# little-little-point-cloud-group/buildingSegment

Measured on AMD Instinct MI355X. Metric: Mpoints/s segmented (kNN+normal+label), higher is better.
Workload: dtype int32 coordinates / f64 normals; 1 GPU; urban_50m; points_per_gpu=50000000, k=16, max_nn=50, rg_mode=0, largest_plane=135921, seed_attempts=6951, fallback_queries=0, rg_rounds=25, validation_rejects=1, tie_rows=971975, parallelism=1 GPU, whole path

## Files before the change

buildingsegment_amd/csrc/bs_grid.hip:

```cpp
#include <hipcub/hipcub.hpp>

#include <algorithm>
#include <climits>
#include <cmath>
#include <cstdio>
#include <cstdlib>

#include "bs_common.h"

namespace bs {

namespace {

__global__ void bbox_kernel(const int32_t* __restrict__ xyz, int64_t n, int32_t* __restrict__ mnmx)
{
  int mn[3] = {INT_MAX, INT_MAX, INT_MAX}, mx[3] = {INT_MIN, INT_MIN, INT_MIN};
  for (int64_t i = blockIdx.x * (int64_t)blockDim.x + threadIdx.x; i < n;
       i += (int64_t)gridDim.x * blockDim.x) {
#pragma unroll
    for (int a = 0; a < 3; a++) {
      int v = xyz[3 * i + a];
      mn[a] = min(mn[a], v);
      mx[a] = max(mx[a], v);
    }
// ... 81 lines not shown
    t[i].end = 0;
  }
}

__global__ void table_insert_kernel(const uint64_t* __restrict__ ukeys, const int32_t* __restrict__ ucnt,
                                    const int32_t* __restrict__ ustart, int32_t ncell, int morton,
                                    CellEntry* table, uint32_t hmask)
{
  int32_t c = blockIdx.x * blockDim.x + threadIdx.x;
  if (c >= ncell)
    return;
  uint64_t k = ukeys[c];
  if (morton)
    k = pack_cell(compact21(k), compact21(k >> 1), compact21(k >> 2));
  uint32_t h = hash_cell(k) & hmask;
  for (;;) {
    unsigned long long prev =
        atomicCAS((unsigned long long*)&table[h].key, ~0ull, (unsigned long long)k);
    if (prev == ~0ull)
      break;
    h = (h + 1) & hmask;
  }
  table[h].start = ustart[c];
  table[h].end = ustart[c] + ucnt[c];
}

__global__ void gather_sorted_kernel(const int32_t* __restrict__ xyz, const int32_t* __restrict__ gidx,
                                     const int32_t* __restrict__ order, int64_t n, int4* __restrict__ spts)
{
  int64_t s = blockIdx.x * (int64_t)blockDim.x + threadIdx.x;
  if (s >= n)
    return;
  int32_t i = order[s];
  int4 v;
  v.x = xyz[3 * (int64_t)i];
  v.y = xyz[3 * (int64_t)i + 1];
  v.z = xyz[3 * (int64_t)i + 2];
  v.w = gidx ? gidx[i] : i;
  spts[s] = v;
}

inline int grid_blocks(int64_t n, int bs) { return (int)((n + bs - 1) / bs); }

}

static int morton_key_bits(int64_t ext, int cell)
{
  int bits = 1;
  while (((int64_t)1 << bits) < ext / cell + 1)
    bits++;
  return std::min(63, 3 * bits);
}

static int sort_count_keys(bs_ctx* ctx, int64_t n, int end_bit, int64_t* ncell)
{
  hipStream_t st = ctx->stream;
  uint64_t* kin = ctx->keys_in.as<uint64_t>();
  uint64_t* kout = ctx->keys_out.as<uint64_t>();
  size_t tb = 0;
  BS_HIP(ctx, hipcub::DeviceRadixSort::SortKeys(nullptr, tb, kin, kout, (int)n, 0, end_bit, st));
  BS_HIP(ctx, ctx->cub_tmp.reserve(tb));
  BS_HIP(ctx, hipcub::DeviceRadixSort::SortKeys(ctx->cub_tmp.p, tb, kin, kout, (int)n, 0, end_bit, st));
  unsigned long long* cnt = ctx->misc.as<unsigned long long>() + 8;
  BS_HIP(ctx, hipMemsetAsync(cnt, 0, sizeof(unsigned long long), st));
  count_heads_kernel<<<std::min(grid_blocks(n, 256), 1024), 256, 0, st>>>(kout, n, cnt);
  unsigned long long h = 0;
  BS_HIP(ctx, hipMemcpyAsync(&h, cnt, sizeof h, hipMemcpyDeviceToHost, st));
  BS_HIP(ctx, hipStreamSynchronize(st));
  *ncell = (int64_t)h;
  return BS_OK;
}

static int count_cells(bs_ctx* ctx, const int32_t* d_xyz, int64_t n, const int mn[3], int cell, int64_t ext,
                       int64_t* ncell)
{
  cellkey_kernel<<<grid_blocks(n, 256), 256, 0, ctx->stream>>>(d_xyz, n, mn[0], mn[1], mn[2], cell, 1,
                                                               ctx->keys_in.as<uint64_t>(), nullptr);
  return sort_count_keys(ctx, n, morton_key_bits(ext, cell), ncell);
}

int build_grid(bs_ctx* ctx, const int32_t* d_xyz, const int32_t* d_gidx, int64_t n, double radius,
               int k, int cell_hint, GridDev* out)
{
  hipStream_t st = ctx->stream;
  if (n <= 0 || n >= (int64_t)INT_MAX - 64)
    return fail(ctx, BS_ERR_INVALID, "point count out of range");
  BS_HIP(ctx, ctx->misc.reserve(256));
  BS_HIP(ctx, ctx->keys_in.reserve(sizeof(uint64_t) * n));
  BS_HIP(ctx, ctx->keys_out.reserve(sizeof(uint64_t) * n));
  BS_HIP(ctx, ctx->vals_in.reserve(sizeof(int32_t) * n));
  BS_HIP(ctx, ctx->vals_out.reserve(sizeof(int32_t) * n));

  int32_t init[6] = {INT_MAX, INT_MAX, INT_MAX, INT_MIN, INT_MIN, INT_MIN};
  int32_t* d_mnmx = ctx->misc.as<int32_t>();
  BS_HIP(ctx, hipMemcpyAsync(d_mnmx, init, sizeof init, hipMemcpyHostToDevice, st));
  bbox_kernel<<<std::min(grid_blocks(n, 256), 512), 256, 0, st>>>(d_xyz, n, d_mnmx);
  int32_t bb[6];
  BS_HIP(ctx, hipMemcpyAsync(bb, d_mnmx, sizeof bb, hipMemcpyDeviceToHost, st));
  BS_HIP(ctx, hipStreamSynchronize(st));
  const int32_t LIM = 1 << 23;
  for (int a = 0; a < 3; a++)
    if (bb[a] <= -LIM || bb[3 + a] >= LIM)
      return fail(ctx, BS_ERR_RANGE, "coordinates must satisfy |c| < 2^23 mm (8.4 km): shift the cloud to its bounding-box origin first "
                                     "(bs_shift_to_origin_dev, or the buildingSeg constructor as TMC3.cpp:210 does)");

  int64_t ext = 1;
  for (int a = 0; a < 3; a++)
    ext = std::max<int64_t>(ext, (int64_t)bb[3 + a] - bb[a] + 1);
  int cell = cell_hint > 0 ? cell_hint : (int)std::max(1.0, std::ceil(radius));
  if (cell_hint <= 0) {
    const double target = std::max(4.0, 0.5 * k);
    const int cmin = cell;
    for (int it = 0; it < 4; it++) {
      int64_t nc = 0;
      int rc = count_cells(ctx, d_xyz, n, bb, cell, ext, &nc);
      if (rc != BS_OK)
        return rc;
      double occ = (double)n / (double)std::max<int64_t>(nc, 1);
      if (occ >= 0.7 * target && occ <= 1.6 * target)
        break;
      double f = std::sqrt(target / occ);
      f = std::min(4.0, std::max(0.25, f));
      int ncell = (int)std::floor(cell * f + 0.5);
      ncell = std::max(ncell, cmin);
      if (ncell == cell || (int64_t)ncell > ext)
        break;
      cell = ncell;
    }
  }
  while (ext / cell + 1 >= (1 << 21))
    cell *= 2;

  uint64_t* kin = ctx->keys_in.as<uint64_t>();
  uint64_t* kout = ctx->keys_out.as<uint64_t>();
  int32_t* vin = ctx->vals_in.as<int32_t>();
  int32_t* vout = ctx->vals_out.as<int32_t>();
  static const int morton = []() {
    const char* e = getenv("BS_GRID_ORDER");
    return (e && e[0] == 'r') ? 0 : 1;
  }();
  cellkey_kernel<<<grid_blocks(n, 256), 256, 0, st>>>(d_xyz, n, bb[0], bb[1], bb[2], cell, morton, kin, vin);
  size_t tb = 0;
  const int end_bit = morton ? morton_key_bits(ext, cell) : 63;
  BS_HIP(ctx, hipcub::DeviceRadixSort::SortPairs(nullptr, tb, kin, kout, vin, vout, (int)n, 0, end_bit, st));
  BS_HIP(ctx, ctx->cub_tmp.reserve(tb));
  BS_HIP(ctx, hipcub::DeviceRadixSort::SortPairs(ctx->cub_tmp.p, tb, kin, kout, vin, vout, (int)n, 0, end_bit, st));

  BS_HIP(ctx, ctx->uniq_keys.reserve(sizeof(uint64_t) * n));
  BS_HIP(ctx, ctx->uniq_cnt.reserve(sizeof(int32_t) * 2 * n));
  uint64_t* ukeys = ctx->uniq_keys.as<uint64_t>();
  int32_t* ucnt = ctx->uniq_cnt.as<int32_t>();
  int32_t* ustart = ucnt + n;
  int32_t* d_nruns = ctx->misc.as<int32_t>() + 32;
  tb = 0;
  BS_HIP(ctx, hipcub::DeviceRunLengthEncode::Encode(nullptr, tb, kout, ukeys, ucnt, d_nruns, (int)n, st));
  BS_HIP(ctx, ctx->cub_tmp.reserve(tb));
  BS_HIP(ctx, hipcub::DeviceRunLengthEncode::Encode(ctx->cub_tmp.p, tb, kout, ukeys, ucnt, d_nruns, (int)n, st));
  int32_t nruns = 0;
  BS_HIP(ctx, hipMemcpyAsync(&nruns, d_nruns, sizeof nruns, hipMemcpyDeviceToHost, st));
  BS_HIP(ctx, hipStreamSynchronize(st));
  if (nruns <= 0)
    return fail(ctx, BS_ERR_INTERNAL, "grid: no occupied cells");
  tb = 0;
  BS_HIP(ctx, hipcub::DeviceScan::ExclusiveSum(nullptr, tb, ucnt, ustart, nruns, st));
  BS_HIP(ctx, ctx->cub_tmp.reserve(tb));
  BS_HIP(ctx, hipcub::DeviceScan::ExclusiveSum(ctx->cub_tmp.p, tb, ucnt, ustart, nruns, st));

  uint32_t hs = 64;
  while (hs < (uint32_t)nruns * 2u)
    hs <<= 1;
  BS_HIP(ctx, ctx->table.reserve(sizeof(CellEntry) * (size_t)hs));
  CellEntry* table = ctx->table.as<CellEntry>();
  table_clear_kernel<<<(hs + 255) / 256, 256, 0, st>>>(table, hs);
  table_insert_kernel<<<(nruns + 255) / 256, 256, 0, st>>>(ukeys, ucnt, ustart, nruns, morton, table, hs - 1);

  BS_HIP(ctx, ctx->spts.reserve(sizeof(int4) * n));
  gather_sorted_kernel<<<grid_blocks(n, 256), 256, 0, st>>>(d_xyz, d_gidx, vout, n, ctx->spts.as<int4>());
  BS_HIP(ctx, hipGetLastError());

  out->mn[0] = bb[0];
  out->mn[1] = bb[1];
  out->mn[2] = bb[2];
  for (int a = 0; a < 3; a++)
    out->dim[a] = (int32_t)(((int64_t)bb[3 + a] - bb[a]) / cell + 1);
  out->cell = cell;
  out->hmask = hs - 1;
  out->table = table;
  out->spts = ctx->spts.as<int4>();
  out->slocal = vout;
  out->n = n;
  ctx->order_n = n;
  ctx->order_xyz = d_xyz;
  return BS_OK;
}

int bbox_dev(bs_ctx* ctx, const int32_t* d_xyz, int64_t n, int32_t bb[6])
{
  hipStream_t st = ctx->stream;
  BS_HIP(ctx, ctx->misc.reserve(256));
// ... 162 lines not shown
                       const int32_t* d_mnmx)
{
  tile_shift_kernel<<<grid_blocks(n, 256), 256, 0, ctx->stream>>>(d_xyz, n, d_off, n_tiles, d_mnmx);
}

int build_grid_tiled(bs_ctx* ctx, const int32_t* d_xyz, const int32_t* d_off, const std::vector<int64_t>& off,
                     double radius, int k, int cell_hint, TiledGridDev* out)
{
  hipStream_t st = ctx->stream;
  const int32_t nt = (int32_t)off.size() - 1;
  const int64_t n = off[nt];
  if (nt < 1 || n <= 0 || n >= (int64_t)INT_MAX - 64)
    return fail(ctx, BS_ERR_INVALID, "point count out of range");
  BS_HIP(ctx, ctx->misc.reserve(256));
  BS_HIP(ctx, ctx->keys_in.reserve(sizeof(uint64_t) * n));
  BS_HIP(ctx, ctx->keys_out.reserve(sizeof(uint64_t) * n));
  BS_HIP(ctx, ctx->vals_in.reserve(sizeof(int32_t) * n));
  BS_HIP(ctx, ctx->vals_out.reserve(sizeof(int32_t) * n));
  BS_HIP(ctx, ctx->bt[BT_MNMX].reserve(sizeof(int32_t) * 6 * nt));
  BS_HIP(ctx, ctx->bt[BT_DESC].reserve(sizeof(TileDesc) * nt));

  std::vector<int32_t> bb;
  int rc = tile_bbox_dev(ctx, d_xyz, d_off, off, ctx->bt[BT_MNMX].as<int32_t>(), bb);
  if (rc != BS_OK)
    return rc;
  const int32_t LIM = 1 << 23;
  int64_t ext = 1;
  for (int32_t t = 0; t < nt; t++)
    for (int a = 0; a < 3; a++) {
      if (bb[6 * t + a] <= -LIM || bb[6 * t + 3 + a] >= LIM) {
        char msg[256];
        snprintf(msg, sizeof msg, "tile %d: coordinates must satisfy |c| < 2^23 mm (8.4 km): shift every tile to its "
                                  "bounding-box origin first (bs_shift_tiles_to_origin_dev)", t);
        return fail(ctx, BS_ERR_RANGE, msg);
      }
      ext = std::max<int64_t>(ext, (int64_t)bb[6 * t + 3 + a] - bb[6 * t + a] + 1);
    }
  int tbits = 0;
  while (((int64_t)1 << tbits) < nt)
    tbits++;
  auto fits = [&](int64_t c) { return ext / c + 1 < (1 << 21) && tbits + morton_key_bits(ext, (int)c) <= 63; };
  std::vector<TileDesc> desc(nt);
  auto upload_desc = [&](int c) -> hipError_t {
    for (int32_t t = 0; t < nt; t++)
      for (int a = 0; a < 3; a++) {
        desc[t].mn[a] = bb[6 * t + a];
        desc[t].dim[a] = (int32_t)(((int64_t)bb[6 * t + 3 + a] - bb[6 * t + a]) / c + 1);
      }
    return hipMemcpyAsync(ctx->bt[BT_DESC].p, desc.data(), sizeof(TileDesc) * nt, hipMemcpyHostToDevice, st);
  };
  BS_HIP(ctx, upload_desc(1));
  const TileDesc* d_desc = ctx->bt[BT_DESC].as<TileDesc>();

  int cell = cell_hint > 0 ? cell_hint : (int)std::max(1.0, std::ceil(radius));
  if (cell_hint <= 0) {
    const double target = std::max(4.0, 0.5 * k);
    const int cmin = cell;
    for (int it = 0; it < 4 && fits(cell); it++) {
      const int mb = morton_key_bits(ext, cell);
      tiled_cellkey_kernel<<<grid_blocks(n, 256), 256, 0, st>>>(d_xyz, n, d_off, nt, d_desc, cell, mb,
                                                                ctx->keys_in.as<uint64_t>(), nullptr);
      int64_t nc = 0;
      rc = sort_count_keys(ctx, n, tbits + mb, &nc);
      if (rc != BS_OK)
        return rc;
      double occ = (double)n / (double)std::max<int64_t>(nc, 1);
      if (occ >= 0.7 * target && occ <= 1.6 * target)
        break;
      double f = std::sqrt(target / occ);
      f = std::min(4.0, std::max(0.25, f));
      int ncell = (int)std::floor(cell * f + 0.5);
      ncell = std::max(ncell, cmin);
      if (ncell == cell || (int64_t)ncell > ext)
        break;
      cell = ncell;
    }
  }
  while (!fits(cell))
    cell *= 2;
  const int mbits = morton_key_bits(ext, cell);
  BS_HIP(ctx, upload_desc(cell));

  uint64_t* kin = ctx->keys_in.as<uint64_t>();
  uint64_t* kout = ctx->keys_out.as<uint64_t>();
  int32_t* vin = ctx->vals_in.as<int32_t>();
  int32_t* vout = ctx->vals_out.as<int32_t>();
  tiled_cellkey_kernel<<<grid_blocks(n, 256), 256, 0, st>>>(d_xyz, n, d_off, nt, d_desc, cell, mbits, kin, vin);
  size_t tb = 0;
  const int end_bit = tbits + mbits;
  BS_HIP(ctx, hipcub::DeviceRadixSort::SortPairs(nullptr, tb, kin, kout, vin, vout, (int)n, 0, end_bit, st));
  BS_HIP(ctx, ctx->cub_tmp.reserve(tb));
  BS_HIP(ctx, hipcub::DeviceRadixSort::SortPairs(ctx->cub_tmp.p, tb, kin, kout, vin, vout, (int)n, 0, end_bit, st));

  BS_HIP(ctx, ctx->uniq_keys.reserve(sizeof(uint64_t) * n));
  BS_HIP(ctx, ctx->uniq_cnt.reserve(sizeof(int32_t) * 2 * n));
  uint64_t* ukeys = ctx->uniq_keys.as<uint64_t>();
  int32_t* ucnt = ctx->uniq_cnt.as<int32_t>();
  int32_t* ustart = ucnt + n;
  int32_t* d_nruns = ctx->misc.as<int32_t>() + 32;
  tb = 0;
  BS_HIP(ctx, hipcub::DeviceRunLengthEncode::Encode(nullptr, tb, kout, ukeys, ucnt, d_nruns, (int)n, st));
  BS_HIP(ctx, ctx->cub_tmp.reserve(tb));
  BS_HIP(ctx, hipcub::DeviceRunLengthEncode::Encode(ctx->cub_tmp.p, tb, kout, ukeys, ucnt, d_nruns, (int)n, st));
  int32_t nruns = 0;
  BS_HIP(ctx, hipMemcpyAsync(&nruns, d_nruns, sizeof nruns, hipMemcpyDeviceToHost, st));
  BS_HIP(ctx, hipStreamSynchronize(st));
  if (nruns <= 0)
    return fail(ctx, BS_ERR_INTERNAL, "grid: no occupied cells");
  tb = 0;
  BS_HIP(ctx, hipcub::DeviceScan::ExclusiveSum(nullptr, tb, ucnt, ustart, nruns, st));
  BS_HIP(ctx, ctx->cub_tmp.reserve(tb));
  BS_HIP(ctx, hipcub::DeviceScan::ExclusiveSum(ctx->cub_tmp.p, tb, ucnt, ustart, nruns, st));

  uint32_t hs = 64;
  while (hs < (uint32_t)nruns * 2u)
    hs <<= 1;
  BS_HIP(ctx, ctx->table.reserve(sizeof(CellEntry) * (size_t)hs));
  CellEntry* table = ctx->table.as<CellEntry>();
  table_clear_kernel<<<(hs + 255) / 256, 256, 0, st>>>(table, hs);
  table_insert_kernel<<<(nruns + 255) / 256, 256, 0, st>>>(ukeys, ucnt, ustart, nruns, 0, table, hs - 1);

  BS_HIP(ctx, ctx->spts.reserve(sizeof(int4) * n));
  gather_sorted_kernel<<<grid_blocks(n, 256), 256, 0, st>>>(d_xyz, nullptr, vout, n, ctx->spts.as<int4>());
  BS_HIP(ctx, hipGetLastError());

  for (int a = 0; a < 3; a++) {
    out->mn[a] = desc[0].mn[a];
    out->dim[a] = desc[0].dim[a];
  }
  out->cell = cell;
  out->hmask = hs - 1;
  out->table = table;
  out->spts = ctx->spts.as<int4>();
  out->slocal = vout;
  out->n = n;
  out->tiles = d_desc;
  out->tile_off = d_off;
  out->n_tiles = nt;
  out->mbits = mbits;
  ctx->order_n = n;
  ctx->order_xyz = d_xyz;
  return BS_OK;
}

}
// ... 1 lines not shown
```

buildingsegment_amd/csrc/bs_knn.hip:

```cpp
#include <cstdlib>
#include <type_traits>

#include "bs_common.h"
#include "bs_normal.h"

namespace bs {

namespace {

constexpr int BS_FAST_RINGS = 2;
constexpr int BS_GENERAL_RINGS = 6;

template <bool TILED>
using GridOf = std::conditional_t<TILED, TiledGridDev, GridDev>;

template <bool TILED>
__device__ inline uint64_t cell_key(uint32_t cx, uint32_t cy, uint32_t cz, uint64_t kbase)
{
  if constexpr (TILED)
    return kbase | morton_cell(cx, cy, cz);
  else
    return pack_cell(cx, cy, cz);
}

__device__ inline void tile_enter(TiledGridDev& g, int64_t s, uint64_t& kbase, int64_t& lo, int64_t& hi)
{
  const int32_t t = tile_of(g.tile_off, g.n_tiles, s);
  const TileDesc d = g.tiles[t];
#pragma unroll
  for (int a = 0; a < 3; a++) {
    g.mn[a] = d.mn[a];
    g.dim[a] = d.dim[a];
  }
  kbase = (uint64_t)t << g.mbits;
  lo = g.tile_off[t];
  hi = g.tile_off[t + 1];
}

template <bool TILED = false>
__device__ inline bool cell_lookup(const GridDev& g, uint32_t cx, uint32_t cy, uint32_t cz, int& start,
                                   int& end, uint64_t kbase = 0)
{
  const uint64_t k = cell_key<TILED>(cx, cy, cz, kbase);
  uint32_t h = hash_cell(k) & g.hmask;
  for (;;) {
    const int4 raw = *reinterpret_cast<const int4*>(&g.table[h]);
    const uint64_t ek = (uint64_t)(uint32_t)raw.x | ((uint64_t)(uint32_t)raw.y << 32);
    if (ek == k) {
      start = raw.z;
      end = raw.w;
      return true;
    }
// ... 135 lines not shown
#pragma unroll
  for (int j = 0; j < KC; j++)
    kth_final = (j == K - 1) ? best[j] : kth_final;
  if (!done || m.n > max_nn || kth_final == ~0ull) {
    const int slot = atomicAdd(fb_count, 1);
    fb_list[slot] = (int32_t)s;
    return;
  }
  int32_t* row = neigh + (int64_t)(loc - q_begin) * K;
#pragma unroll
  for (int j = 0; j < KC; j++)
    if (j < K)
      row[j] = (int32_t)(uint32_t)best[j];
  if (npos) {
    int32_t* prow = npos + s * K;
#pragma unroll
    for (int j = 0; j < KC; j++)
      if (j < K)
        prow[j] = bpos[j];
  }
  if (normals) {
    const V3 nv = normal_from_moments(m);
    double* o = normals + 3 * (int64_t)(loc - q_begin);
    o[0] = nv.x;
    o[1] = nv.y;
    o[2] = nv.z;
    if (npos) {
      double* po = pnorm_of(npos, g.n, K) + 3 * s;
      po[0] = nv.x;
      po[1] = nv.y;
      po[2] = nv.z;
    }
  }
  if (cert_r2 && (kth_final >> 32) >= cert_r2)
    atomicAdd(uncert, 1ull);
  if (tie_rows) {
    bool tie = false;
    uint64_t next = runner;
#pragma unroll
    for (int j = 0; j + 1 < KC; j++) {
      tie = tie || (j + 1 < K && (best[j] >> 32) == (best[j + 1] >> 32));
      next = (j + 1 == K) ? best[j + 1] : next;
    }
    tie = tie || (next != ~0ull && (next >> 32) == (kth_final >> 32));
    if (tie)
      atomicAdd(tie_rows, 1ull);
  }
}

#ifndef BS_KNN_CAP4
#define BS_KNN_CAP4 0
#endif
constexpr int KBUF = 8;

template <int KC, bool REL32, bool TILED = false>
__global__ __launch_bounds__(256) __attribute__((amdgpu_waves_per_eu(KC == 16 && REL32 && BS_KNN_CAP4 ? 4 : 2))) void knn_fast2_kernel(GridOf<TILED> g, int64_t q_begin, int64_t q_end, int K,
                                                       int max_nn, double r2, int32_t* __restrict__ neigh,
                                                       double* __restrict__ normals,
                                                       int32_t* __restrict__ fb_list,
                                                       int32_t* __restrict__ fb_count, uint64_t cert_r2,
                                                       unsigned long long* __restrict__ uncert,
                                                       int32_t* __restrict__ npos, unsigned long long* __restrict__ tie_rows)
{
  const int64_t s = xcd_logical_block() * (int64_t)blockDim.x + threadIdx.x;
  if (s >= g.n)
    return;
  const int32_t loc = g.slocal[s];
  if (loc < q_begin || loc >= q_end)
    return;
  uint64_t kbase = 0;
  if constexpr (TILED) {
    int64_t lo, hi;
    tile_enter(g, s, kbase, lo, hi);
  }
  uint64_t runner = ~0ull;
  const int4 P = g.spts[s];
  const int q[3] = {P.x, P.y, P.z};
  const int ci[3] = {(int)((uint32_t)(P.x - g.mn[0]) / (uint32_t)g.cell),
                     (int)((uint32_t)(P.y - g.mn[1]) / (uint32_t)g.cell),
                     (int)((uint32_t)(P.z - g.mn[2]) / (uint32_t)g.cell)};
  __shared__ uint32_t blo[KBUF][256], bhi[KBUF][256];
  __shared__ int bps[KBUF][256];
  int nbuf = 0;
  uint64_t best[KC];
  int bpos[KC];
#pragma unroll
  for (int j = 0; j < KC; j++) {
    best[j] = ~0ull;
    bpos[j] = 0;
  }
  Moments m = {};
  int rsx = 0, rsy = 0, rsz = 0, rsxx = 0, rsyy = 0, rszz = 0, rsxy = 0, rsxz = 0, rsyz = 0, rn = 0;
  bool done = false;
  auto flush = [&]() {
    uint64_t bk[KBUF];
    int bp[KBUF];
#pragma unroll
    for (int i = 0; i < KBUF; i++) {
      const bool have = i < nbuf;
      bk[i] = have ? (((uint64_t)bhi[i][threadIdx.x] << 32) | blo[i][threadIdx.x]) : ~0ull;
      bp[i] = have ? bps[i][threadIdx.x] : 0;
    }
    nbuf = 0;
#define BS_CE(ka, pa, kb, pb)            \
  do {                                   \
    const bool sw_ = (kb) < (ka);        \
    const uint64_t tk_ = (ka);           \
    const int tp_ = (pa);                \
    (ka) = sw_ ? (kb) : (ka);            \
    (pa) = sw_ ? (pb) : (pa);            \
    (kb) = sw_ ? tk_ : (kb);             \
    (pb) = sw_ ? tp_ : (pb);             \
  } while (0)
    constexpr int net[19][2] = {{0, 1}, {2, 3}, {4, 5}, {6, 7}, {0, 2}, {1, 3}, {4, 6}, {5, 7}, {1, 2}, {5, 6},
                                {0, 4}, {3, 7}, {1, 5}, {2, 6}, {1, 4}, {3, 6}, {2, 4}, {3, 5}, {3, 4}};
#pragma unroll
    for (int c = 0; c < 19; c++)
      BS_CE(bk[net[c][0]], bp[net[c][0]], bk[net[c][1]], bp[net[c][1]]);
#pragma unroll
    for (int i = 0; i < KBUF; i++)
      BS_CE(best[KC - KBUF + i], bpos[KC - KBUF + i], bk[KBUF - 1 - i], bp[KBUF - 1 - i]);
#pragma unroll
    for (int i = 0; i < KBUF; i++)
      runner = bk[i] < runner ? bk[i] : runner;
#pragma unroll
    for (int d = KC / 2; d >= 1; d >>= 1) {
#pragma unroll
      for (int i = 0; i < KC; i++)
        if ((i & d) == 0)
          BS_CE(best[i], bpos[i], best[i + d], bpos[i + d]);
    }
#undef BS_CE
  };
  for (int rho = 0; rho <= BS_FAST_RINGS && !done; rho++) {
    for (int dz = -rho; dz <= rho; dz++) {
      const int cz = ci[2] + dz;
      if (cz < 0 || cz >= g.dim[2])
        continue;
      for (int dy = -rho; dy <= rho; dy++) {
        const int cy = ci[1] + dy;
        if (cy < 0 || cy >= g.dim[1])
          continue;
        const bool face = (dz == -rho || dz == rho || dy == -rho || dy == rho);
        const int step = face ? 1 : (rho > 0 ? 2 * rho : 1);
        for (int dx0 = -rho; dx0 <= rho; dx0 += 3 * step) {
          int4 raw[3];
          uint64_t ck[3];
          uint32_t hh[3];
          bool want[3];
#pragma unroll
          for (int u = 0; u < 3; u++) {
            const int dx = dx0 + u * step;
            const int cx = ci[0] + dx;
            want[u] = dx <= rho && cx >= 0 && cx < g.dim[0];
            ck[u] = cell_key<TILED>((uint32_t)(want[u] ? cx : ci[0]), (uint32_t)cy, (uint32_t)cz, kbase);
            hh[u] = hash_cell(ck[u]) & g.hmask;
            raw[u] = *reinterpret_cast<const int4*>(&g.table[hh[u]]);
          }
          int cs3[3], ce3[3];
#pragma unroll
          for (int u = 0; u < 3; u++) {
            cs3[u] = 0;
            ce3[u] = 0;
            if (!want[u])
              continue;
            for (;;) {
              const uint64_t ek = (uint64_t)(uint32_t)raw[u].x | ((uint64_t)(uint32_t)raw[u].y << 32);
              if (ek == ck[u]) {
                cs3[u] = raw[u].z;
                ce3[u] = raw[u].w;
                break;
              }
              if (ek == ~0ull)
                break;
              hh[u] = (hh[u] + 1) & g.hmask;
              raw[u] = *reinterpret_cast<const int4*>(&g.table[hh[u]]);
            }
          }
#pragma unroll 1
          for (int u = 0; u < 3; u++) {
            const int cs = u == 0 ? cs3[0] : (u == 1 ? cs3[1] : cs3[2]);
            const int ce = u == 0 ? ce3[0] : (u == 1 ? ce3[1] : ce3[2]);
            for (int t0 = cs; t0 < ce; t0 += 4) {
              int4 cc[4];
#pragma unroll
              for (int v = 0; v < 4; v++)
                cc[v] = g.spts[t0 + v < ce ? t0 + v : ce - 1];
#pragma unroll
              for (int v = 0; v < 4; v++) {
                const int t = t0 + v;
                const int4 c = cc[v];
                const int ex = c.x - q[0], ey = c.y - q[1], ez = c.z - q[2];
                const uint32_t d2 = (uint32_t)(ex * ex) + (uint32_t)(ey * ey) + (uint32_t)(ez * ez);
                const uint64_t key = ((uint64_t)d2 << 32) | (uint32_t)c.w;
                const bool real = t < ce;
                if (real && key < best[KC - 1]) {
                  blo[nbuf][threadIdx.x] = (uint32_t)key;
                  bhi[nbuf][threadIdx.x] = d2;
                  bps[nbuf][threadIdx.x] = t;
                  nbuf++;
                } else if (real) {
                  runner = key < runner ? key : runner;
                }
                if (__ballot(nbuf == KBUF))
                  flush();
                if (real && (double)d2 < r2) {
                  if constexpr (REL32) {
                    rsx += ex;
                    rsy += ey;
                    rsz += ez;
                    rsxx += __mul24(ex, ex);
                    rsyy += __mul24(ey, ey);
                    rszz += __mul24(ez, ez);
                    rsxy += __mul24(ex, ey);
                    rsxz += __mul24(ex, ez);
                    rsyz += __mul24(ey, ez);
                    rn += 1;
                  } else {
                    moments_add(m, c.x, c.y, c.z);
                  }
                }
              }
            }
          }
        }
      }
    }
    if (__ballot(nbuf > 0))
      flush();
    uint64_t R2;
    const bool bounded = guaranteed_radius(g, q, ci, rho, R2);
    if (!bounded) {
      done = true;
    } else {
      uint64_t kth = ~0ull;
#pragma unroll
      for (int j = 0; j < KC; j++)
        kth = (j == K - 1) ? best[j] : kth;
      const bool knn_ok = kth != ~0ull && (kth >> 32) < R2;
      const bool nrm_ok = (double)R2 >= r2;
      done = knn_ok && nrm_ok;
    }
  }
  uint64_t kth_final = ~0ull;
#pragma unroll
  for (int j = 0; j < KC; j++)
    kth_final = (j == K - 1) ? best[j] : kth_final;
  if constexpr (REL32) {
    const int64_t n64 = rn, qx = q[0], qy = q[1], qz = q[2];
    m.n = rn;
    m.sx = n64 * qx + rsx;
    m.sy = n64 * qy + rsy;
    m.sz = n64 * qz + rsz;
    m.sxx = (uint64_t)(n64 * qx * qx + 2 * qx * rsx + rsxx);
    m.syy = (uint64_t)(n64 * qy * qy + 2 * qy * rsy + rsyy);
    m.szz = (uint64_t)(n64 * qz * qz + 2 * qz * rsz + rszz);
    m.sxy = n64 * qx * qy + qx * rsy + qy * rsx + rsxy;
    m.sxz = n64 * qx * qz + qx * rsz + qz * rsx + rsxz;
    m.syz = n64 * qy * qz + qy * rsz + qz * rsy + rsyz;
  }
  if (!done || m.n > max_nn || kth_final == ~0ull) {
    const int slot = atomicAdd(fb_count, 1);
    fb_list[slot] = (int32_t)s;
    return;
  }
  int32_t* row = neigh + (int64_t)(loc - q_begin) * K;
#pragma unroll
  for (int j = 0; j < KC; j++)
    if (j < K)
      row[j] = (int32_t)(uint32_t)best[j];
  if (npos) {
    int32_t* prow = npos + s * K;
#pragma unroll
    for (int j = 0; j < KC; j++)
      if (j < K)
        prow[j] = bpos[j];
  }
  if (normals) {
    const V3 nv = normal_from_moments(m);
    double* o = normals + 3 * (int64_t)(loc - q_begin);
    o[0] = nv.x;
    o[1] = nv.y;
    o[2] = nv.z;
    if (npos) {
      double* po = pnorm_of(npos, g.n, K) + 3 * s;
      po[0] = nv.x;
      po[1] = nv.y;
      po[2] = nv.z;
    }
  }
  if (cert_r2 && (kth_final >> 32) >= cert_r2)
    atomicAdd(uncert, 1ull);
  if (tie_rows) {
    bool tie = false;
    uint64_t next = runner;
#pragma unroll
// ... 321 lines not shown
        bool tie = count > K && bd2[K] == bd2[K - 1];
        for (int j = 0; j + 1 < K; j++)
          tie = tie || bd2[j] == bd2[j + 1];
        if (tie)
          atomicAdd(tie_rows, 1ull);
      }
    }
    __syncthreads();
  }
}

__global__ void mark_all_kernel(GridDev g, int64_t q_begin, int64_t q_end, int32_t* fb_list,
                                int32_t* fb_count)
{
  const int64_t s = blockIdx.x * (int64_t)blockDim.x + threadIdx.x;
  if (s >= g.n)
    return;
  const int32_t loc = g.slocal[s];
  if (loc < q_begin || loc >= q_end)
    return;
  fb_list[atomicAdd(fb_count, 1)] = (int32_t)s;
}

}

template <bool TILED>
static int launch_knn(bs_ctx* ctx, const GridOf<TILED>& g, int64_t q_begin, int64_t q_end, const bs_params& p,
                      int32_t* d_neigh, double* d_normals, double cert_radius, int64_t* n_uncertified, int32_t* d_npos)
{
  hipStream_t st = ctx->stream;
  const int64_t n = g.n;
  BS_HIP(ctx, ctx->fb_list.reserve(sizeof(int32_t) * (2 * n + 32)));
  int32_t* fb_list = ctx->fb_list.as<int32_t>() + 16;
  int32_t* fb_count = ctx->fb_list.as<int32_t>();
  int32_t* fb2_list = fb_list + n + 16;
  int32_t* fb2_count = ctx->fb_list.as<int32_t>() + 2;
  unsigned long long* uncert = (unsigned long long*)(ctx->fb_list.as<int32_t>() + 4);
  unsigned long long* tie_rows = (unsigned long long*)(ctx->fb_list.as<int32_t>() + 8);
  BS_HIP(ctx, hipMemsetAsync(ctx->fb_list.p, 0, 64, st));
  const double r2 = p.radius * p.radius;
  uint64_t cert_r2 = 0;
  if (cert_radius > 0) {
    double c2 = cert_radius * cert_radius;
    cert_r2 = c2 >= 1.8e19 ? ~0ull : (uint64_t)std::ceil(c2);
    if (cert_r2 == 0)
      cert_r2 = 1;
  }
  const int blocks = (int)((n + 255) / 256);
  const int xblocks = xcd_grid(blocks);
  const bool fast_ok = (int64_t)g.cell * (2 * BS_FAST_RINGS + 1) <= 37500;
  if (fast_ok) {
    const bool buffered = getenv("BS_KNN_BUFFERED") ? atoi(getenv("BS_KNN_BUFFERED")) != 0 : true;
    const bool rel32 = r2 <= 32761.0 && !getenv("BS_KNN_MOMENTS64");
    if (buffered && p.k <= 16 && rel32)
      knn_fast2_kernel<16, true, TILED><<<xblocks, 256, 0, st>>>(g, q_begin, q_end, p.k, p.max_nn, r2, d_neigh, d_normals,
                                                         fb_list, fb_count, cert_r2, uncert, d_npos, tie_rows);
    else if (buffered && p.k <= 16)
      knn_fast2_kernel<16, false, TILED><<<xblocks, 256, 0, st>>>(g, q_begin, q_end, p.k, p.max_nn, r2, d_neigh, d_normals,
                                                          fb_list, fb_count, cert_r2, uncert, d_npos, tie_rows);
    else if (buffered && rel32)
      knn_fast2_kernel<32, true, TILED><<<xblocks, 256, 0, st>>>(g, q_begin, q_end, p.k, p.max_nn, r2, d_neigh, d_normals,
                                                         fb_list, fb_count, cert_r2, uncert, d_npos, tie_rows);
    else if (buffered)
      knn_fast2_kernel<32, false, TILED><<<xblocks, 256, 0, st>>>(g, q_begin, q_end, p.k, p.max_nn, r2, d_neigh, d_normals,
                                                          fb_list, fb_count, cert_r2, uncert, d_npos, tie_rows);
    else if (p.k <= 16)
      knn_fast_kernel<16, TILED><<<xblocks, 256, 0, st>>>(g, q_begin, q_end, p.k, p.max_nn, r2, d_neigh, d_normals,
                                                  fb_list, fb_count, cert_r2, uncert, d_npos, tie_rows);
    else
      knn_fast_kernel<32, TILED><<<xblocks, 256, 0, st>>>(g, q_begin, q_end, p.k, p.max_nn, r2, d_neigh, d_normals,
                                                  fb_list, fb_count, cert_r2, uncert, d_npos, tie_rows);
  } else {
    mark_all_kernel<<<blocks, 256, 0, st>>>(g, q_begin, q_end, fb_list, fb_count);
  }
  if (getenv("BS_KNN_GENERAL_THREAD")) {
    knn_general_kernel<TILED><<<1024, 64, 0, st>>>(g, q_begin, p.k, p.max_nn, r2, d_neigh, d_normals, fb_list, fb_count, cert_r2,
                                            uncert, d_npos, tie_rows);
  } else {
    knn_general_wave_kernel<TILED><<<8192, 64, 0, st>>>(g, q_begin, p.k, p.max_nn, r2, d_neigh, d_normals, fb_list, fb_count, cert_r2,
                                                 uncert, d_npos, tie_rows, fb2_list, fb2_count);
    knn_general_kernel<TILED><<<1024, 64, 0, st>>>(g, q_begin, p.k, p.max_nn, r2, d_neigh, d_normals, fb2_list, fb2_count, cert_r2,
                                            uncert, d_npos, tie_rows);
  }
  BS_HIP(ctx, hipGetLastError());
  int32_t hb[4];
  BS_HIP(ctx, hipMemcpyAsync(hb, ctx->fb_list.p, sizeof hb, hipMemcpyDeviceToHost, st));
  unsigned long long hu = 0, ht = 0;
  BS_HIP(ctx, hipMemcpyAsync(&hu, uncert, sizeof hu, hipMemcpyDeviceToHost, st));
  BS_HIP(ctx, hipMemcpyAsync(&ht, tie_rows, sizeof ht, hipMemcpyDeviceToHost, st));
  BS_HIP(ctx, hipStreamSynchronize(st));
  ctx->tm.n_fallback_queries = hb[0];
  ctx->tm.tie_rows = (int64_t)ht;
  if (n_uncertified)
    *n_uncertified = (int64_t)hu;
  return BS_OK;
}

int launch_knn_normals(bs_ctx* ctx, const GridDev& g, int64_t q_begin, int64_t q_end, const bs_params& p,
                       int32_t* d_neigh, double* d_normals, double cert_radius, int64_t* n_uncertified, int32_t* d_npos)
{
  return launch_knn<false>(ctx, g, q_begin, q_end, p, d_neigh, d_normals, cert_radius, n_uncertified, d_npos);
}

int launch_knn_normals_tiled(bs_ctx* ctx, const TiledGridDev& g, const bs_params& p, int32_t* d_neigh,
                             double* d_normals, int32_t* d_npos)
{
  return launch_knn<true>(ctx, g, 0, g.n, p, d_neigh, d_normals, 0.0, nullptr, d_npos);
}

}
```

Before: 199.2 Mpoints/s.

## Stream ring-1 kNN cells as one candidate queue and reuse grid-sizing sort

In the buffered kNN kernel, the ring-1 neighborhood is processed per z-slab. All 9 hash lookups are issued up front, the non-empty cell ranges are stored in shared memory, and their candidates are consumed as one continuous stream of 4-wide batches that cross cell boundaries. This is meant to cut the wave divergence and idle lanes caused by short per-cell loops, at the cost of extra shared memory and a changed occupancy hint (waves_per_eu 3). Separately, grid building now sorts key/value pairs from the second cell-size probe onward, so if the last probe's cell size is the final one, the final cellkey and radix sort are skipped. The in-radius test also switches from a double comparison to a precomputed integer threshold.

```diff
diff --git a/buildingsegment_amd/csrc/bs_grid.hip b/buildingsegment_amd/csrc/bs_grid.hip
--- a/buildingsegment_amd/csrc/bs_grid.hip
+++ b/buildingsegment_amd/csrc/bs_grid.hip
@@ -157,15 +157,23 @@
   return std::min(63, 3 * bits);
 }
 
-static int sort_count_keys(bs_ctx* ctx, int64_t n, int end_bit, int64_t* ncell)
+static int sort_count_keys(bs_ctx* ctx, int64_t n, int end_bit, int64_t* ncell, bool pairs)
 {
   hipStream_t st = ctx->stream;
   uint64_t* kin = ctx->keys_in.as<uint64_t>();
   uint64_t* kout = ctx->keys_out.as<uint64_t>();
+  int32_t* vin = ctx->vals_in.as<int32_t>();
+  int32_t* vout = ctx->vals_out.as<int32_t>();
   size_t tb = 0;
-  BS_HIP(ctx, hipcub::DeviceRadixSort::SortKeys(nullptr, tb, kin, kout, (int)n, 0, end_bit, st));
-  BS_HIP(ctx, ctx->cub_tmp.reserve(tb));
-  BS_HIP(ctx, hipcub::DeviceRadixSort::SortKeys(ctx->cub_tmp.p, tb, kin, kout, (int)n, 0, end_bit, st));
+  if (pairs) {
+    BS_HIP(ctx, hipcub::DeviceRadixSort::SortPairs(nullptr, tb, kin, kout, vin, vout, (int)n, 0, end_bit, st));
+    BS_HIP(ctx, ctx->cub_tmp.reserve(tb));
+    BS_HIP(ctx, hipcub::DeviceRadixSort::SortPairs(ctx->cub_tmp.p, tb, kin, kout, vin, vout, (int)n, 0, end_bit, st));
+  } else {
+    BS_HIP(ctx, hipcub::DeviceRadixSort::SortKeys(nullptr, tb, kin, kout, (int)n, 0, end_bit, st));
+    BS_HIP(ctx, ctx->cub_tmp.reserve(tb));
+    BS_HIP(ctx, hipcub::DeviceRadixSort::SortKeys(ctx->cub_tmp.p, tb, kin, kout, (int)n, 0, end_bit, st));
+  }
   unsigned long long* cnt = ctx->misc.as<unsigned long long>() + 8;
   BS_HIP(ctx, hipMemsetAsync(cnt, 0, sizeof(unsigned long long), st));
   count_heads_kernel<<<std::min(grid_blocks(n, 256), 1024), 256, 0, st>>>(kout, n, cnt);
@@ -177,11 +185,18 @@
 }
 
 static int count_cells(bs_ctx* ctx, const int32_t* d_xyz, int64_t n, const int mn[3], int cell, int64_t ext,
-                       int64_t* ncell)
+                       int64_t* ncell, bool pairs)
 {
   cellkey_kernel<<<grid_blocks(n, 256), 256, 0, ctx->stream>>>(d_xyz, n, mn[0], mn[1], mn[2], cell, 1,
-                                                               ctx->keys_in.as<uint64_t>(), nullptr);
-  return sort_count_keys(ctx, n, morton_key_bits(ext, cell), ncell);
+                                                               ctx->keys_in.as<uint64_t>(),
+                                                               pairs ? ctx->vals_in.as<int32_t>() : nullptr);
+  return sort_count_keys(ctx, n, morton_key_bits(ext, cell), ncell, pairs);
+}
+
+static bool grid_reuse_on()
+{
+  const char* e = getenv("BS_GRID_REUSE");
+  return !e || atoi(e) != 0;
 }
 
 int build_grid(bs_ctx* ctx, const int32_t* d_xyz, const int32_t* d_gidx, int64_t n, double radius,
@@ -212,15 +227,23 @@
   int64_t ext = 1;
   for (int a = 0; a < 3; a++)
     ext = std::max<int64_t>(ext, (int64_t)bb[3 + a] - bb[a] + 1);
+  static const int morton = []() {
+    const char* e = getenv("BS_GRID_ORDER");
+    return (e && e[0] == 'r') ? 0 : 1;
+  }();
+  const bool reuse = morton && grid_reuse_on();
+  int sorted_cell = 0;
   int cell = cell_hint > 0 ? cell_hint : (int)std::max(1.0, std::ceil(radius));
   if (cell_hint <= 0) {
     const double target = std::max(4.0, 0.5 * k);
     const int cmin = cell;
     for (int it = 0; it < 4; it++) {
       int64_t nc = 0;
-      int rc = count_cells(ctx, d_xyz, n, bb, cell, ext, &nc);
+      const bool pairs = reuse && it >= 1;
+      int rc = count_cells(ctx, d_xyz, n, bb, cell, ext, &nc, pairs);
       if (rc != BS_OK)
         return rc;
+      sorted_cell = pairs ? cell : 0;
       double occ = (double)n / (double)std::max<int64_t>(nc, 1);
       if (occ >= 0.7 * target && occ <= 1.6 * target)
         break;
@@ -240,16 +263,14 @@
   uint64_t* kout = ctx->keys_out.as<uint64_t>();
   int32_t* vin = ctx->vals_in.as<int32_t>();
   int32_t* vout = ctx->vals_out.as<int32_t>();
-  static const int morton = []() {
-    const char* e = getenv("BS_GRID_ORDER");
-    return (e && e[0] == 'r') ? 0 : 1;
-  }();
-  cellkey_kernel<<<grid_blocks(n, 256), 256, 0, st>>>(d_xyz, n, bb[0], bb[1], bb[2], cell, morton, kin, vin);
   size_t tb = 0;
-  const int end_bit = morton ? morton_key_bits(ext, cell) : 63;
-  BS_HIP(ctx, hipcub::DeviceRadixSort::SortPairs(nullptr, tb, kin, kout, vin, vout, (int)n, 0, end_bit, st));
-  BS_HIP(ctx, ctx->cub_tmp.reserve(tb));
-  BS_HIP(ctx, hipcub::DeviceRadixSort::SortPairs(ctx->cub_tmp.p, tb, kin, kout, vin, vout, (int)n, 0, end_bit, st));
+  if (sorted_cell != cell) {
+    cellkey_kernel<<<grid_blocks(n, 256), 256, 0, st>>>(d_xyz, n, bb[0], bb[1], bb[2], cell, morton, kin, vin);
+    const int end_bit = morton ? morton_key_bits(ext, cell) : 63;
+    BS_HIP(ctx, hipcub::DeviceRadixSort::SortPairs(nullptr, tb, kin, kout, vin, vout, (int)n, 0, end_bit, st));
+    BS_HIP(ctx, ctx->cub_tmp.reserve(tb));
+    BS_HIP(ctx, hipcub::DeviceRadixSort::SortPairs(ctx->cub_tmp.p, tb, kin, kout, vin, vout, (int)n, 0, end_bit, st));
+  }
 
   BS_HIP(ctx, ctx->uniq_keys.reserve(sizeof(uint64_t) * n));
   BS_HIP(ctx, ctx->uniq_cnt.reserve(sizeof(int32_t) * 2 * n));
@@ -518,18 +539,23 @@
   BS_HIP(ctx, upload_desc(1));
   const TileDesc* d_desc = ctx->bt[BT_DESC].as<TileDesc>();
 
+  const bool reuse = grid_reuse_on();
+  int sorted_cell = 0;
   int cell = cell_hint > 0 ? cell_hint : (int)std::max(1.0, std::ceil(radius));
   if (cell_hint <= 0) {
     const double target = std::max(4.0, 0.5 * k);
     const int cmin = cell;
     for (int it = 0; it < 4 && fits(cell); it++) {
       const int mb = morton_key_bits(ext, cell);
+      const bool pairs = reuse && it >= 1;
       tiled_cellkey_kernel<<<grid_blocks(n, 256), 256, 0, st>>>(d_xyz, n, d_off, nt, d_desc, cell, mb,
-                                                                ctx->keys_in.as<uint64_t>(), nullptr);
+                                                                ctx->keys_in.as<uint64_t>(),
+                                                                pairs ? ctx->vals_in.as<int32_t>() : nullptr);
       int64_t nc = 0;
-      rc = sort_count_keys(ctx, n, tbits + mb, &nc);
+      rc = sort_count_keys(ctx, n, tbits + mb, &nc, pairs);
       if (rc != BS_OK)
         return rc;
+      sorted_cell = pairs ? cell : 0;
       double occ = (double)n / (double)std::max<int64_t>(nc, 1);
       if (occ >= 0.7 * target && occ <= 1.6 * target)
         break;
@@ -551,12 +577,14 @@
   uint64_t* kout = ctx->keys_out.as<uint64_t>();
   int32_t* vin = ctx->vals_in.as<int32_t>();
   int32_t* vout = ctx->vals_out.as<int32_t>();
-  tiled_cellkey_kernel<<<grid_blocks(n, 256), 256, 0, st>>>(d_xyz, n, d_off, nt, d_desc, cell, mbits, kin, vin);
   size_t tb = 0;
-  const int end_bit = tbits + mbits;
-  BS_HIP(ctx, hipcub::DeviceRadixSort::SortPairs(nullptr, tb, kin, kout, vin, vout, (int)n, 0, end_bit, st));
-  BS_HIP(ctx, ctx->cub_tmp.reserve(tb));
-  BS_HIP(ctx, hipcub::DeviceRadixSort::SortPairs(ctx->cub_tmp.p, tb, kin, kout, vin, vout, (int)n, 0, end_bit, st));
+  if (sorted_cell != cell) {
+    tiled_cellkey_kernel<<<grid_blocks(n, 256), 256, 0, st>>>(d_xyz, n, d_off, nt, d_desc, cell, mbits, kin, vin);
+    const int end_bit = tbits + mbits;
+    BS_HIP(ctx, hipcub::DeviceRadixSort::SortPairs(nullptr, tb, kin, kout, vin, vout, (int)n, 0, end_bit, st));
+    BS_HIP(ctx, ctx->cub_tmp.reserve(tb));
+    BS_HIP(ctx, hipcub::DeviceRadixSort::SortPairs(ctx->cub_tmp.p, tb, kin, kout, vin, vout, (int)n, 0, end_bit, st));
+  }
 
   BS_HIP(ctx, ctx->uniq_keys.reserve(sizeof(uint64_t) * n));
   BS_HIP(ctx, ctx->uniq_cnt.reserve(sizeof(int32_t) * 2 * n));
diff --git a/buildingsegment_amd/csrc/bs_knn.hip b/buildingsegment_amd/csrc/bs_knn.hip
--- a/buildingsegment_amd/csrc/bs_knn.hip
+++ b/buildingsegment_amd/csrc/bs_knn.hip
@@ -1,3 +1,6 @@
+#include <algorithm>
+#include <cmath>
+#include <cstdio>
 #include <cstdlib>
 #include <type_traits>
 
@@ -239,10 +242,16 @@
 #define BS_KNN_CAP4 0
 #endif
 constexpr int KBUF = 8;
-
-template <int KC, bool REL32, bool TILED = false>
-__global__ __launch_bounds__(256) __attribute__((amdgpu_waves_per_eu(KC == 16 && REL32 && BS_KNN_CAP4 ? 4 : 2))) void knn_fast2_kernel(GridOf<TILED> g, int64_t q_begin, int64_t q_end, int K,
-                                                       int max_nn, double r2, int32_t* __restrict__ neigh,
+#ifndef BS_KNN_PROBE_GROUP
+#define BS_KNN_PROBE_GROUP 3
+#endif
+#ifdef BS_PROBE
+__device__ unsigned long long g_knn_probe[8];
+#endif
+
+template <int KC, bool REL32, bool TILED = false, bool STREAM = false>
+__global__ __launch_bounds__(256) __attribute__((amdgpu_waves_per_eu(KC == 16 && REL32 && BS_KNN_CAP4 ? 4 : (KC == 16 && REL32 && STREAM ? 3 : 2)))) void knn_fast2_kernel(GridOf<TILED> g, int64_t q_begin, int64_t q_end, int K,
+                                                       int max_nn, double r2, uint32_t r2le, int32_t* __restrict__ neigh,
                                                        double* __restrict__ normals,
                                                        int32_t* __restrict__ fb_list,
                                                        int32_t* __restrict__ fb_count, uint64_t cert_r2,
@@ -268,6 +277,7 @@
                      (int)((uint32_t)(P.z - g.mn[2]) / (uint32_t)g.cell)};
   __shared__ uint32_t blo[KBUF][256], bhi[KBUF][256];
   __shared__ int bps[KBUF][256];
+  __shared__ int srs[STREAM ? 9 : 1][STREAM ? 256 : 1], sre[STREAM ? 9 : 1][STREAM ? 256 : 1];
   int nbuf = 0;
   uint64_t best[KC];
   int bpos[KC];
@@ -279,7 +289,7 @@
   Moments m = {};
   int rsx = 0, rsy = 0, rsz = 0, rsxx = 0, rsyy = 0, rszz = 0, rsxy = 0, rsxz = 0, rsyz = 0, rn = 0;
   bool done = false;
-  auto flush = [&]() {
+  auto flush = [&]() __attribute__((always_inline)) {
     uint64_t bk[KBUF];
     int bp[KBUF];
 #pragma unroll
@@ -319,8 +329,154 @@
     }
 #undef BS_CE
   };
+  auto cand_slot = [&](const int4 c, const int t, const bool real) __attribute__((always_inline)) {
+    const int ex = c.x - q[0], ey = c.y - q[1], ez = c.z - q[2];
+    const uint32_t d2 = (uint32_t)(ex * ex) + (uint32_t)(ey * ey) + (uint32_t)(ez * ez);
+    const uint64_t key = ((uint64_t)d2 << 32) | (uint32_t)c.w;
+    if (real && key < best[KC - 1]) {
+      blo[nbuf][threadIdx.x] = (uint32_t)key;
+      bhi[nbuf][threadIdx.x] = d2;
+      bps[nbuf][threadIdx.x] = t;
+      nbuf++;
+    } else if (real) {
+      runner = key < runner ? key : runner;
+    }
+    if (__ballot(nbuf == KBUF))
+      flush();
+    if (real && d2 <= r2le) {
+      if constexpr (REL32) {
+        rsx += ex;
+        rsy += ey;
+        rsz += ez;
+        rsxx += __mul24(ex, ex);
+        rsyy += __mul24(ey, ey);
+        rszz += __mul24(ez, ez);
+        rsxy += __mul24(ex, ey);
+        rsxz += __mul24(ex, ez);
+        rsyz += __mul24(ey, ez);
+        rn += 1;
+      } else {
+        moments_add(m, c.x, c.y, c.z);
+      }
+    }
+  };
+#ifdef BS_PROBE
+  int probe_exec = 0, probe_cand = 0;
+#define BS_PROBE_BATCH()                                                         \
+  do {                                                                           \
+    if (rho <= 1 && (int)(threadIdx.x & 63) == __ffsll((long long)__ballot(1)) - 1) \
+      probe_exec++;                                                              \
+  } while (0)
+#define BS_PROBE_CELL(cnt) \
+  do {                     \
+    if (rho <= 1)          \
+      probe_cand += (cnt); \
+  } while (0)
+#else
+#define BS_PROBE_BATCH() \
+  do {                   \
+  } while (0)
+#define BS_PROBE_CELL(cnt) \
+  do {                     \
+  } while (0)
+#endif
   for (int rho = 0; rho <= BS_FAST_RINGS && !done; rho++) {
-    for (int dz = -rho; dz <= rho; dz++) {
+    const bool streamed = STREAM && rho == 1;
+    if (streamed) {
+#pragma unroll 1
+      for (int dz = -1; dz <= 1; dz++) {
+        const int cz = ci[2] + dz;
+        const bool zok = cz >= 0 && cz < g.dim[2];
+        int cnt = 0;
+        constexpr int GP = BS_KNN_PROBE_GROUP;
+        static_assert(9 % GP == 0, "probe groups tile the slab");
+#pragma unroll
+        for (int u0 = 0; u0 < 9; u0 += GP) {
+          int4 raw[GP];
+          uint64_t ck[GP];
+          uint32_t hh[GP];
+          bool want[GP];
+#pragma unroll
+          for (int w = 0; w < GP; w++) {
+            const int u = u0 + w;
+            const int cy = ci[1] + u / 3 - 1, cx = ci[0] + u % 3 - 1;
+            want[w] = zok && cy >= 0 && cy < g.dim[1] && cx >= 0 && cx < g.dim[0] && !(dz == 0 && u == 4);
+            ck[w] = cell_key<TILED>((uint32_t)(want[w] ? cx : ci[0]), (uint32_t)(want[w] ? cy : ci[1]),
+                                    (uint32_t)(want[w] ? cz : ci[2]), kbase);
+            hh[w] = hash_cell(ck[w]) & g.hmask;
+            raw[w] = *reinterpret_cast<const int4*>(&g.table[hh[w]]);
+          }
+#pragma unroll
+          for (int w = 0; w < GP; w++) {
+            int cs = 0, ce = 0;
+            if (want[w]) {
+              for (;;) {
+                const uint64_t ek = (uint64_t)(uint32_t)raw[w].x | ((uint64_t)(uint32_t)raw[w].y << 32);
+                if (ek == ck[w]) {
+                  cs = raw[w].z;
+                  ce = raw[w].w;
+                  break;
+                }
+                if (ek == ~0ull)
+                  break;
+                hh[w] = (hh[w] + 1) & g.hmask;
+                raw[w] = *reinterpret_cast<const int4*>(&g.table[hh[w]]);
+              }
+            }
+            BS_PROBE_CELL(ce - cs);
+            if (cs < ce) {
+              srs[cnt][threadIdx.x] = cs;
+              sre[cnt][threadIdx.x] = ce;
+              cnt++;
+            }
+          }
+        }
+        int cur = 0;
+        int t0 = cnt > 0 ? srs[0][threadIdx.x] : 0, e0 = cnt > 0 ? sre[0][threadIdx.x] : 0;
+        int s1 = cnt > 1 ? srs[1][threadIdx.x] : 0, e1 = cnt > 1 ? sre[1][threadIdx.x] : 0;
+        while (t0 < e0) {
+          BS_PROBE_BATCH();
+          const int rem = e0 - t0;
+          int ta[4];
+          bool rl[4];
+          int4 cc[4];
+#pragma unroll
+          for (int v = 0; v < 4; v++) {
+            const int t1 = s1 + (v - rem);
+            rl[v] = v < rem || t1 < e1;
+            ta[v] = v < rem ? t0 + v : t1;
+            cc[v] = g.spts[rl[v] ? ta[v] : (int)s];
+          }
+#pragma unroll
+          for (int v = 0; v < 4; v++)
+            cand_slot(cc[v], ta[v], rl[v]);
+          const bool pop1 = rem <= 4;
+          t0 += pop1 ? 0 : 4;
+          if (__ballot(pop1)) {
+            const bool more1 = pop1 && cur + 2 < cnt;
+            const int i2 = min(cur + 2, 8);
+            const int s2 = more1 ? srs[i2][threadIdx.x] : 0, e2 = more1 ? sre[i2][threadIdx.x] : 0;
+            t0 = pop1 ? s1 + (4 - rem) : t0;
+            e0 = pop1 ? e1 : e0;
+            s1 = pop1 ? s2 : s1;
+            e1 = pop1 ? e2 : e1;
+            cur += pop1 ? 1 : 0;
+            const bool pop2 = pop1 && e0 != 0 && t0 >= e0;
+            if (__ballot(pop2)) {
+              const bool more2 = pop2 && cur + 2 < cnt;
+              const int i3 = min(cur + 2, 8);
+              const int s3 = more2 ? srs[i3][threadIdx.x] : 0, e3 = more2 ? sre[i3][threadIdx.x] : 0;
+              t0 = pop2 ? s1 : t0;
+              e0 = pop2 ? e1 : e0;
+              s1 = pop2 ? s3 : s1;
+              e1 = pop2 ? e3 : e1;
+              cur += pop2 ? 1 : 0;
+            }
+          }
+        }
+      }
+    }
+    for (int dz = -rho; !streamed && dz <= rho; dz++) {
       const int cz = ci[2] + dz;
       if (cz < 0 || cz >= g.dim[2])
         continue;
@@ -368,46 +524,16 @@
           for (int u = 0; u < 3; u++) {
             const int cs = u == 0 ? cs3[0] : (u == 1 ? cs3[1] : cs3[2]);
             const int ce = u == 0 ? ce3[0] : (u == 1 ? ce3[1] : ce3[2]);
+            BS_PROBE_CELL(ce - cs);
             for (int t0 = cs; t0 < ce; t0 += 4) {
+              BS_PROBE_BATCH();
               int4 cc[4];
 #pragma unroll
               for (int v = 0; v < 4; v++)
                 cc[v] = g.spts[t0 + v < ce ? t0 + v : ce - 1];
 #pragma unroll
-              for (int v = 0; v < 4; v++) {
-                const int t = t0 + v;
-                const int4 c = cc[v];
-                const int ex = c.x - q[0], ey = c.y - q[1], ez = c.z - q[2];
-                const uint32_t d2 = (uint32_t)(ex * ex) + (uint32_t)(ey * ey) + (uint32_t)(ez * ez);
-                const uint64_t key = ((uint64_t)d2 << 32) | (uint32_t)c.w;
-                const bool real = t < ce;
-                if (real && key < best[KC - 1]) {
-                  blo[nbuf][threadIdx.x] = (uint32_t)key;
-                  bhi[nbuf][threadIdx.x] = d2;
-                  bps[nbuf][threadIdx.x] = t;
-                  nbuf++;
-                } else if (real) {
-                  runner = key < runner ? key : runner;
-                }
-                if (__ballot(nbuf == KBUF))
-                  flush();
-                if (real && (double)d2 < r2) {
-                  if constexpr (REL32) {
-                    rsx += ex;
-                    rsy += ey;
-                    rsz += ez;
-                    rsxx += __mul24(ex, ex);
-                    rsyy += __mul24(ey, ey);
-                    rszz += __mul24(ez, ez);
-                    rsxy += __mul24(ex, ey);
-                    rsxz += __mul24(ex, ez);
-                    rsyz += __mul24(ey, ez);
-                    rn += 1;
-                  } else {
-                    moments_add(m, c.x, c.y, c.z);
-                  }
-                }
-              }
+              for (int v = 0; v < 4; v++)
+                cand_slot(cc[v], t0 + v, t0 + v < ce);
             }
           }
         }
@@ -429,6 +555,31 @@
       done = knn_ok && nrm_ok;
     }
   }
+#undef BS_PROBE_BATCH
+#undef BS_PROBE_CELL
+#ifdef BS_PROBE
+  {
+    const unsigned long long act = __ballot(1);
+    const int lane = threadIdx.x & 63;
+    const int need = (probe_cand + 3) / 4;
+    int ex_sum = probe_exec, nd_max = need, nd_sum = need, ln = 1;
+    for (int o = 32; o > 0; o >>= 1) {
+      const int a = __shfl_xor(ex_sum, o), b = __shfl_xor(nd_max, o), c = __shfl_xor(nd_sum, o), d = __shfl_xor(ln, o);
+      const bool ok = (act >> (lane ^ o)) & 1;
+      ex_sum += ok ? a : 0;
+      nd_max = ok && b > nd_max ? b : nd_max;
+      nd_sum += ok ? c : 0;
+      ln += ok ? d : 0;
+    }
+    if (lane == __ffsll((long long)act) - 1) {
+      atomicAdd(&g_knn_probe[0], (unsigned long long)ex_sum);
+      atomicAdd(&g_knn_probe[1], (unsigned long long)nd_max);
+      atomicAdd(&g_knn_probe[2], (unsigned long long)nd_sum);
+      atomicAdd(&g_knn_probe[3], (unsigned long long)ln);
+      atomicAdd(&g_knn_probe[4], 1ull);
+    }
+  }
+#endif
   uint64_t kth_final = ~0ull;
 #pragma unroll
   for (int j = 0; j < KC; j++)
@@ -856,18 +1007,28 @@
   if (fast_ok) {
     const bool buffered = getenv("BS_KNN_BUFFERED") ? atoi(getenv("BS_KNN_BUFFERED")) != 0 : true;
     const bool rel32 = r2 <= 32761.0 && !getenv("BS_KNN_MOMENTS64");
+    const bool stream = (getenv("BS_KNN_STREAM") ? atoi(getenv("BS_KNN_STREAM")) != 0 : true) && !(TILED && p.k <= 16 && !rel32);
+    const uint32_t r2le = (uint32_t)(std::min(std::ceil(r2), 4294967296.0) - 1.0);
+#define BS_FAST2(KC_, REL_)                                                                                              \
+  do {                                                                                                                   \
+    if (stream)                                                                                                          \
+      knn_fast2_kernel<KC_, REL_, TILED, true><<<xblocks, 256, 0, st>>>(g, q_begin, q_end, p.k, p.max_nn, r2, r2le, d_neigh, \
+                                                                        d_normals, fb_list, fb_count, cert_r2, uncert,  \
+                                                                        d_npos, tie_rows);                              \
+    else                                                                                                                 \
+      knn_fast2_kernel<KC_, REL_, TILED, false><<<xblocks, 256, 0, st>>>(g, q_begin, q_end, p.k, p.max_nn, r2, r2le, d_neigh, \
+                                                                         d_normals, fb_list, fb_count, cert_r2, uncert, \
+                                                                         d_npos, tie_rows);                             \
+  } while (0)
     if (buffered && p.k <= 16 && rel32)
-      knn_fast2_kernel<16, true, TILED><<<xblocks, 256, 0, st>>>(g, q_begin, q_end, p.k, p.max_nn, r2, d_neigh, d_normals,
-                                                         fb_list, fb_count, cert_r2, uncert, d_npos, tie_rows);
+      BS_FAST2(16, true);
     else if (buffered && p.k <= 16)
-      knn_fast2_kernel<16, false, TILED><<<xblocks, 256, 0, st>>>(g, q_begin, q_end, p.k, p.max_nn, r2, d_neigh, d_normals,
-                                                          fb_list, fb_count, cert_r2, uncert, d_npos, tie_rows);
+      BS_FAST2(16, false);
     else if (buffered && rel32)
-      knn_fast2_kernel<32, true, TILED><<<xblocks, 256, 0, st>>>(g, q_begin, q_end, p.k, p.max_nn, r2, d_neigh, d_normals,
-                                                         fb_list, fb_count, cert_r2, uncert, d_npos, tie_rows);
+      BS_FAST2(32, true);
     else if (buffered)
-      knn_fast2_kernel<32, false, TILED><<<xblocks, 256, 0, st>>>(g, q_begin, q_end, p.k, p.max_nn, r2, d_neigh, d_normals,
-                                                          fb_list, fb_count, cert_r2, uncert, d_npos, tie_rows);
+      BS_FAST2(32, false);
+#undef BS_FAST2
     else if (p.k <= 16)
       knn_fast_kernel<16, TILED><<<xblocks, 256, 0, st>>>(g, q_begin, q_end, p.k, p.max_nn, r2, d_neigh, d_normals,
                                                   fb_list, fb_count, cert_r2, uncert, d_npos, tie_rows);
@@ -893,6 +1054,18 @@
   BS_HIP(ctx, hipMemcpyAsync(&hu, uncert, sizeof hu, hipMemcpyDeviceToHost, st));
   BS_HIP(ctx, hipMemcpyAsync(&ht, tie_rows, sizeof ht, hipMemcpyDeviceToHost, st));
   BS_HIP(ctx, hipStreamSynchronize(st));
+#ifdef BS_PROBE
+  {
+    unsigned long long pr[8] = {};
+    BS_HIP(ctx, hipMemcpyFromSymbol(pr, HIP_SYMBOL(g_knn_probe), sizeof pr));
+    if (pr[4])
+      fprintf(stderr, "knn probe: waves %llu lanes %llu executed batches/wave %.2f largest need/wave %.2f mean need/lane %.2f "
+                      "executed/largest %.3f\n", pr[4], pr[3], (double)pr[0] / pr[4], (double)pr[1] / pr[4],
+              (double)pr[2] / pr[3], (double)pr[0] / (double)pr[1]);
+    const unsigned long long zero[8] = {};
+    BS_HIP(ctx, hipMemcpyToSymbol(HIP_SYMBOL(g_knn_probe), zero, sizeof zero));
+  }
+#endif
   ctx->tm.n_fallback_queries = hb[0];
   ctx->tm.tie_rows = (int64_t)ht;
   if (n_uncertified)
```

After: 202.3 Mpoints/s (median of 6 runs). 1.6% higher.
